# jwang1x/VT-precondition

Measured on AMD Instinct MI355X. Metric: precond-GMRES iters/sec + CSR SpMV achieved-HBM-GB/s, 1/2/4/8 MI355X, higher is better.
Workload: dtype f64; 1 GPU; C3: GMRES(20, auto)+BJ(8) to rtol=1e-08, n=20000000, row-sharded over 1 GPU(s); n=20000000, nnz=99950000, restart=20, prec=bj, bs=8, operator=generated, line_band=800, bj_apply=tridiag, layout=sell, orth=auto, parallelism=row-slab x1

## Files before the change

vt-precondition_amd/csrc/vtk_band.hip:

```cpp
#include <hip/hip_runtime.h>

#include <algorithm>
#include <cstdlib>

#include "vtk_device.hpp"

namespace vtk {


#define VTK_BAND_DOTS_UNROLL 2
constexpr int BAND_XUP_XB = 4;
constexpr int BAND_PF = 12;

template <int OPT> constexpr int band_wpe() { return (OPT & 2) ? 6 : 4; }
__device__ __forceinline__ int band_block(int opt, int H) {
    const int b = blockIdx.x;
    if (!(opt & 4) || H != 2 || (gridDim.x & 15) != 0) return b;
    return (((b >> 4) << 3) + (b & 7)) * 2 + ((b >> 3) & 1);
}
__device__ __forceinline__ double band_msub(double acc, double a, double b) { return __builtin_fma(-a, b, acc); }
__device__ __forceinline__ double band_madd(double acc, double a, double b) { return __builtin_fma(a, b, acc); }
template <int OPT> __device__ __forceinline__ void band_sync() {
    if constexpr (OPT & 8) asm volatile("s_waitcnt lgkmcnt(0)\n\ts_barrier" ::: "memory");
    else __syncthreads();
}
constexpr int BAND_OFF = 16;
static_assert(BAND_LP + 2 * BAND_OFF <= BAND_T && BAND_OFF % 8 == 0, "band geometry");
template <int WU, int J, int VMODE = 0, bool GH = true, int OPT = 0>
__global__ __launch_bounds__(BAND_T) __attribute__((amdgpu_waves_per_eu(band_wpe<OPT>()))) void k_band_step(BandK a) {
    constexpr int BAND_RS = BAND_T;
    constexpr int BAND_W = BAND_T / 64, BAND_IT = (J + 2 + BAND_W - 1) / BAND_W;
    __shared__ double vbuf[(J + 1) * BAND_LP];
    __shared__ double ring[4 * BAND_RS];
    __shared__ double wbuf[BAND_LP];
    __shared__ double red[DC_NQ];
    __shared__ double cs[BAND_JV], ce[BAND_JV], cp[BAND_JV];
    __shared__ int pf_sink[64];
    constexpr int j = J;
    if (__builtin_nontemporal_load(&a.st->xup_tag) == j) {
        dc_xupdate_body<BAND_XUP_XB, true>(a.V, a.ld, j, __builtin_nontemporal_load(&a.st->stop_col), a.n, a.cf, a.x,
                                           a.H, a.S, a.m, a.w_prev);
        return;
    }
    if (stopped(&a.st->stop_col, j)) return;
    const int tid = threadIdx.x, lane = tid & 63, wv = tid >> 6;
    const int L = a.L, X = a.X, H = a.H_parts, LP = L / H;
    const int b = band_block(a.opt, H), R = (int)gridDim.x / H, rb = b / H, h = b % H, v0 = h * LP;
    const int xa = (int)((int64_t)rb * X / R), xb = (int)((int64_t)(rb + 1) * X / R);
    const int v = v0 - BAND_OFF + tid;
    const int wrapL = (X - 1) * L;
    const bool own = tid >= BAND_OFF && tid < BAND_OFF + LP;
    const bool upd = tid >= BAND_OFF - 1 && tid <= LP + BAND_OFF && v >= 0 && v < L;
    constexpr bool LSV = VMODE >= 1, CANON = VMODE == 2;
    const int ii = lane & 7;
    double tx0 = 0.0, tx1 = 0.0;
    if constexpr (LSV) {
        if (v >= 0 && v < L) {
            tx0 = a.lsv[a.n + v];
            tx1 = a.lsv[a.n + L + v];
        }
    }
    for (int k = tid; k < j; k += BAND_T) {
        cs[k] = a.cf->s[k];
        ce[k] = a.cf->e[k];
        cp[k] = a.cf->e_prev[k];
    }
    const double rinv = a.cf->rinv, qc = a.cf->q, ej = a.cf->e[j], qp = a.cf->q_prev;
    band_sync<OPT>();
    double vreg[J + 1];
    double acc[BAND_IT][3];
#pragma unroll
    for (int u = 0; u < BAND_IT; ++u) acc[u][0] = acc[u][1] = acc[u][2] = 0.0;
    const int nl = xb - xa;
    const int xhm = xa == 0 ? X - 1 : xa - 1, xhp = xb == X ? 0 : xb;
    const bool rev = ((a.opt & 16) && (rb & 1)) != ((a.opt & 32) && (J & 1));
    auto line_of = [&](int it, int &kind) {
        if (rev) {
            kind = it == 0 ? 2 : (it == nl + 1 ? 1 : 0);
            return it == 0 ? xhp : (it == nl + 1 ? xhm : xb - it);
        }
        kind = it == 0 ? 1 : (it == nl + 1 ? 2 : 0);
        return it == 0 ? xhm : (it == nl + 1 ? xhp : xa - 1 + it);
    };
    auto spmv_line = [&](int it) { return rev ? xb + 1 - it : xa - 2 + it; };
    constexpr bool PF = J <= BAND_PF;
    constexpr bool SPF = PF && CANON && (OPT & 1);
    struct Ld {
        double v[J > 0 ? J : 1];
        double wm, wj;
        double drow, mrow, tv0, tv1;
    };
    auto load = [&](int it, Ld &o) {
        int kind;
        const int y = line_of(it, kind);
        if constexpr (SPF) {
            o.drow = 0.0;
            o.mrow = 1.0;
            o.tv0 = o.tv1 = 0.0;
            if (it >= 2) {
                const int xs = spmv_line(it);
                const int64_t rs = (int64_t)xs * L + (own ? v : v0);
                if (own) {
                    o.drow = __builtin_nontemporal_load(a.lsv + rs);
                    o.mrow = __builtin_nontemporal_load(a.mtri + rs);
                }
                o.tv0 = a.lsv[a.n + 2 * L + xs];
                o.tv1 = a.lsv[a.n + 2 * L + X + xs];
            }
        }
        const int64_t row = (int64_t)y * L + (upd ? v : 0);
        o.wm = 0.0;
        o.wj = 0.0;
        const double *gh = (GH && a.ghost && ((kind == 1 && rb == 0) || (kind == 2 && rb == R - 1)))
                               ? a.ghost + (size_t)(kind == 1 ? 0 : 1) * (a.m + 2) * L : nullptr;
        if (upd) {
            if (gh) {
                o.wj = gh[(size_t)(a.m + (j & 1)) * L + v];
                o.wm = gh[(size_t)(j == 0 ? 0 : a.m + ((j + 1) & 1)) * L + v];
            } else {
                o.wj = __builtin_nontemporal_load(a.w_in + row);
                o.wm = __builtin_nontemporal_load((j == 0 ? a.V : a.w_prev) + row);
            }
        }
        if (gh) {
#pragma unroll
            for (int k = 0; k < J; ++k) o.v[k] = upd ? gh[(size_t)k * L + v] : 0.0;
        } else {
            const double *pv = a.V + row;
#pragma unroll
            for (int k = 0; k < J; ++k) {
                o.v[k] = upd ? __builtin_nontemporal_load(pv) : 0.0;
                pv += a.ld;
            }
        }
    };
    auto update = [&](int it, const Ld &o) -> double {
        int kind;
        const int y = line_of(it, kind);
        const int64_t row = (int64_t)y * L + (upd ? v : 0);
#pragma unroll
        for (int k = 0; k < J; ++k) vreg[k] = o.v[k];
        double pj = o.wm;
        if (j >= 1) {
            double tp = o.wm;
#pragma unroll
            for (int k = 0; k < J; ++k) tp = band_msub(tp, cp[k], vreg[k]);
            pj = tp * qp;
        }
        double av = pj, tv = o.wj;
#pragma unroll
        for (int k = 0; k < J; ++k) {
            const double sk = cs[k], ek = ce[k];
            av = band_msub(av, sk, vreg[k]);
            tv = band_msub(tv, ek, vreg[k]);
        }
        double vj = pj;
        if (j >= 1) vj = av * rinv;
        tv = band_msub(tv, ej, vj);
        const double pn = tv * qc;
        vreg[J] = vj;
        if (kind == 0 && own) {
            if (j >= 1) {
                st_wt(a.V + (size_t)j * a.ld + row, vj);
            }
            if (j == a.m - 2) st_wt(a.V + (size_t)(j + 1) * a.ld + row, pn);
        }
        return pn;
    };
    auto stage = [&](double *vb) {
        if (own) {
#pragma unroll
            for (int k = 0; k <= J; ++k) vb[k * BAND_LP + tid - BAND_OFF] = vreg[k];
        }
    };
    auto slot = [&](int y) { return ((y - xa + 1) & 3) * BAND_RS; };
    constexpr int PF_ROWS = J + 2 + (CANON ? 2 : 0);
    auto l2_prefetch = [&](int itp) {
        if constexpr ((OPT & 8) != 0) {
            if (itp > nl + 1) return;
            int kind;
            const int y = line_of(itp, kind);
            const bool ghostl = GH && a.ghost && ((kind == 1 && rb == 0) || (kind == 2 && rb == R - 1));
            const int xs = spmv_line(itp);
            const int vlo = v0 > 0 ? v0 - 1 : 0, vhi = v0 + LP < L ? v0 + LP + 1 : L;
            for (int r = wv; r < PF_ROWS; r += BAND_W) {
                const double *vec;
                int64_t r0, r1;
                if (r < J + 2) {
                    if (ghostl) continue;
                    vec = r < J ? a.V + (size_t)r * a.ld : (r == J ? a.w_in : (j == 0 ? a.V : a.w_prev));
                    r0 = (int64_t)y * L + vlo;
                    r1 = (int64_t)y * L + vhi;
                } else {
                    if (itp < 2) continue;
                    vec = r == J + 2 ? a.lsv : a.mtri;
                    r0 = (int64_t)xs * L + v0;
                    r1 = r0 + LP;
                }
                const int64_t s0 = r0 >> 4, ns = ((r1 - 1) >> 4) - s0 + 1;
                if (lane < ns)
                    __builtin_amdgcn_global_load_lds(vec + ((s0 + lane) << 4), (__attribute__((address_space(3))) void *)pf_sink,
                                                     4, 0, 0);
            }
        }
    };
    Ld nx;
    if constexpr (PF) load(0, nx);
    l2_prefetch(PF ? 1 : 0);
    for (int it = 0; it <= nl + 1; ++it) {
        const int y = rev ? xb - it : xa - 1 + it, x = spmv_line(it);
        const bool work = it >= 2;
        const int64_t lrow = (int64_t)(work ? x : xa) * L;
        const int64_t row = lrow + (own ? v : v0);
        const int64_t q = row >> 6, q0 = (lrow + v0 - BAND_OFF + 64 * wv) >> 6;
        const int l64 = (int)(row & 63);
        uint32_t word = 0u;
        int dv = 0;
        double d[LSV ? 1 : WU];
        double mrow = 1.0, drow = 0.0, tv0 = 0.0, tv1 = 0.0;
        if (work && !SPF) {
            if constexpr (!CANON) {
                word = __builtin_nontemporal_load(a.pk + q * 64 + l64);
                const int64_t qd = q0 + (lane >> 4);
                dv = (lane < 32 && qd >= 0 && qd * 64 < a.n) ? a.dict[qd * 16 + (lane & 15)] : 0;
            }
            if constexpr (LSV) {
                if (own) drow = __builtin_nontemporal_load(a.lsv + row);
                tv0 = a.lsv[a.n + 2 * L + x];
                tv1 = a.lsv[a.n + 2 * L + X + x];
            } else {
#pragma unroll
                for (int k = 0; k < WU; ++k) d[k] = __builtin_nontemporal_load(a.val + q * 64 * WU + 64 * k + l64);
            }
            if (own) mrow = __builtin_nontemporal_load(a.mtri + row);
        }
        {
            Ld cu;
            if constexpr (PF) cu = nx;
            else load(it, cu);
            if constexpr (SPF) {
                drow = cu.drow;
                mrow = cu.mrow;
                tv0 = cu.tv0;
                tv1 = cu.tv1;
            }
            const double pn = update(it, cu);
            if (upd) ring[slot(y) + tid] = pn;
            if constexpr (PF) {
                if (it <= nl) load(it + 1, nx);
            }
            l2_prefetch(PF ? it + 2 : it + 1);
        }
        band_sync<OPT>();
        if (work) {
            double sacc = 0.0, sub = 0.0, sup = 0.0;
            if constexpr (CANON) {
                int64_t cxm, cxp;
                const int ord = __builtin_amdgcn_readfirstlane(
                    canon_order_xv(x, 0, a.n, L, X, GH && a.ghost ? a.left_blk : -1, cxm, cxp, a.xord));
                const int sx = ((x - xa + 1) & 3) * BAND_RS - v0 + BAND_OFF;
                constexpr int P_MID = 0 | 1 << 3 | 2 << 6 | 3 << 9 | 4 << 12;
                constexpr int P_FIRST = 1 | 2 << 3 | 3 << 6 | 4 << 9 | 0 << 12;
                constexpr int P_LAST = 4 | 0 << 3 | 1 << 6 | 2 << 9 | 3 << 12;
                const bool sl = a.canon == 2 && (ord == P_MID || ord == P_FIRST || ord == P_LAST);
                if (sl) {
                    const int vv = own ? v : v0;
                    const double t0 = tx0 * ring[((x - xa) & 3) * BAND_RS - v0 + BAND_OFF + vv];
                    const double t4 = tx1 * ring[((x - xa + 2) & 3) * BAND_RS - v0 + BAND_OFF + vv];
                    const double t2 = drow * ring[sx + vv];
                    const double t1 = tv0 * ring[sx + vv - 1];
                    const double t3 = tv1 * ring[sx + vv + 1];
                    const bool h1 = vv > 0, h3 = vv < L - 1;
                    double sa = 0.0;
                    if (ord == P_MID) {
                        sa = sa + t0;
                        sa = h1 ? sa + t1 : sa;
                        sa = sa + t2;
                        sa = h3 ? sa + t3 : sa;
                        sa = sa + t4;
                    } else if (ord == P_FIRST) {
                        sa = h1 ? sa + t1 : sa;
                        sa = sa + t2;
                        sa = h3 ? sa + t3 : sa;
                        sa = sa + t4;
                        sa = sa + t0;
                    } else {
                        sa = sa + t4;
                        sa = sa + t0;
                        sa = h1 ? sa + t1 : sa;
                        sa = sa + t2;
                        sa = h3 ? sa + t3 : sa;
                    }
                    sacc = own ? sa : 0.0;
                    sub = (own && h1 && ii > 0) ? 0.0 + tv0 : 0.0;
                    sup = (own && h3 && ii < 7) ? 0.0 + tv1 : 0.0;
                }
#pragma unroll
                for (int e = 0; e < 5; ++e) {
                    const int kind = (ord >> (3 * e)) & 7;
                    if (!sl && own) {
                        if (kind == 0) sacc += tx0 * ring[((x - xa) & 3) * BAND_RS - v0 + BAND_OFF + v];
                        else if (kind == 4) sacc += tx1 * ring[((x - xa + 2) & 3) * BAND_RS - v0 + BAND_OFF + v];
                        else if (kind == 2) sacc += drow * ring[sx + v];
                        else if (kind == 1) {
                            if (v > 0) {
                                sacc += tv0 * ring[sx + v - 1];
                                if (ii > 0) sub = sub + tv0;
                            }
                        } else if (v < L - 1) {
                            sacc += tv1 * ring[sx + v + 1];
                            if (ii < 7) sup = sup + tv1;
                        }
                    }
                }
            } else {
                const int sel = (int)(q - q0) * 16;
#pragma unroll
                for (int k = 0; k < WU; ++k) {
                    const int code = (int)((word >> (4 * k)) & 15u);
                    const int off = __shfl(dv, (sel + code) & 63, 64);
                    if (own && code != PK_CODES) {
                        const int t = v + off;
                        int rel, vc;
                        const int c = x * L + t;
                        if (a.ghost && c >= (int)a.n) {
                            const int kk = c - (int)a.n, blk = kk >= L ? 1 : 0;
                            rel = blk == a.left_blk ? -1 : 1;
                            vc = kk - blk * L;
                        } else if (t >= 0 && t < L) { rel = 0; vc = t; }
                        else if (t >= L && t < 2 * L) { rel = 1; vc = t - L; }
                        else if (t < 0 && t >= -L) { rel = -1; vc = t + L; }
                        else if (t >= L) { rel = -1; vc = t - wrapL; }
                        else { rel = 1; vc = t + wrapL; }
                        const double xv = ring[((x - xa + 1 + rel) & 3) * BAND_RS + vc - v0 + BAND_OFF];
                        double dk;
                        if constexpr (LSV) dk = rel != 0 ? (rel > 0 ? tx1 : tx0) : (vc == v ? drow : (vc > v ? tv1 : tv0));
                        else dk = d[k];
                        sacc += dk * xv;
                        if (off == -1 && ii > 0) sub = sub + dk;
                        if (off == 1 && ii < 7) sup = sup + dk;
                    }
                }
            }
            const double z = bj_trim_group<8>(own ? sacc : 0.0, lane, sub, sup, mrow);
            if (own) {
                st_wt(a.w_out + row, z);
                wbuf[tid - BAND_OFF] = z;
            }
            band_sync<OPT>();
            const double *pr = ring + slot(x) + BAND_OFF;
#pragma unroll
            for (int u = 0; u < BAND_IT; ++u) {
                const int itm = wv + BAND_W * u;
                if (itm <= j) {
                    const double *vk = vbuf + itm * BAND_LP;
#pragma unroll VTK_BAND_DOTS_UNROLL
                    for (int t = lane; t < LP; t += 64) {
                        const double vv = vk[t];
                        acc[u][0] = band_madd(acc[u][0], vv, pr[t]);
                        acc[u][1] = band_madd(acc[u][1], vv, wbuf[t]);
                    }
                } else if (itm == j + 1) {
#pragma unroll VTK_BAND_DOTS_UNROLL
                    for (int t = lane; t < LP; t += 64) {
                        const double pv = pr[t], wq = wbuf[t];
                        acc[u][0] = band_madd(acc[u][0], pv, pv);
                        acc[u][1] = band_madd(acc[u][1], pv, wq);
                        acc[u][2] = band_madd(acc[u][2], wq, wq);
                    }
                }
            }
            band_sync<OPT>();
        }
        if (it >= 1 && it <= nl) stage(vbuf);
    }
#pragma unroll
    for (int u = 0; u < BAND_IT; ++u) {
        const int itm = wv + BAND_W * u;
        if (itm <= j + 1) {
            const double t0 = wave_allsum(acc[u][0]), t1 = wave_allsum(acc[u][1]), t2 = wave_allsum(acc[u][2]);
            if (lane == 0) {
                if (itm <= j) {
                    red[itm] = t0;
                    red[DC_MAXJ + itm] = t1;
                } else {
                    red[2 * DC_MAXJ] = t0;
                    red[2 * DC_MAXJ + 1] = t1;
                    red[2 * DC_MAXJ + 2] = t2;
                }
            }
        }
    }
    __syncthreads();
    const int jn = j + 1;
    for (int qq = tid; qq < DC_NQ; qq += BAND_T) {
        const bool used = qq < jn || (qq >= DC_MAXJ && qq < DC_MAXJ + jn) || qq >= 2 * DC_MAXJ;
        if (used) a.part[(size_t)qq * GMAX + b] = red[qq];
    }
}

template <int J> constexpr bool band_spf_j() { return J == 0 || J == 3 || J == 4; }
template <int J> static void launch_band_one_rank(const BandK &a0, int grid, hipStream_t s) {
    BandK a = a0;
    if constexpr (!band_spf_j<J>()) a.opt &= ~1;
    const dim3 g(grid), blk(BAND_T);
    if constexpr (J > BAND_PF) {
        if (a.opt & 8) { hipLaunchKernelGGL((k_band_step<5, J, 2, false, 9>), g, blk, 0, s, a); return; }
    }
    if constexpr (J <= BAND_J3) {
        if ((a.opt & 3) == 3) { hipLaunchKernelGGL((k_band_step<5, J, 2, false, 3>), g, blk, 0, s, a); return; }
        if ((a.opt & 3) == 2) { hipLaunchKernelGGL((k_band_step<5, J, 2, false, 2>), g, blk, 0, s, a); return; }
    }
    if (a.opt & 1) hipLaunchKernelGGL((k_band_step<5, J, 2, false, 1>), g, blk, 0, s, a);
    else hipLaunchKernelGGL((k_band_step<5, J, 2, false>), g, blk, 0, s, a);
}

template <int J> static void launch_band_ghost(const BandK &a0, int grid, hipStream_t s) {
    BandK a = a0;
    if constexpr (!band_spf_j<J>()) a.opt &= ~1;
    const dim3 g(grid), blk(BAND_T);
    if constexpr (J > BAND_PF) {
        if (a.opt & 8) { hipLaunchKernelGGL((k_band_step<5, J, 2, true, 9>), g, blk, 0, s, a); return; }
    }
    if constexpr (J <= BAND_J3) {
        if ((a.opt & 3) == 3) { hipLaunchKernelGGL((k_band_step<5, J, 2, true, 3>), g, blk, 0, s, a); return; }
        if ((a.opt & 3) == 2) { hipLaunchKernelGGL((k_band_step<5, J, 2, true, 2>), g, blk, 0, s, a); return; }
    }
    if constexpr (J > BAND_J3 && J <= BAND_PF) {
        if (a.opt & 1) { hipLaunchKernelGGL((k_band_step<5, J, 2, true, 1>), g, blk, 0, s, a); return; }
    }
    hipLaunchKernelGGL((k_band_step<5, J, 2>), g, blk, 0, s, a);
}

hipError_t launch_band_step(const BandK &a, int grid, int wu, hipStream_t s) {
    if (wu != 5 || a.H_parts < 1 || a.L % a.H_parts != 0 || a.L / a.H_parts > BAND_LP || (a.L / a.H_parts) % 8 != 0 ||
        a.j + 1 > BAND_JV || grid < a.H_parts || grid > GMAX || grid % a.H_parts != 0 || grid / a.H_parts > a.X ||
        a.n > INT32_MAX / 2)
        return hipErrorInvalidValue;
    switch (a.j) {
#define VTK_BAND_J(J_)                                                                                           \
    case J_:                                                                                                     \
        if (a.lsv && a.canon && !a.ghost) launch_band_one_rank<J_>(a, grid, s); \
        else if (a.lsv && a.canon) launch_band_ghost<J_>(a, grid, s); \
        else if (a.lsv) hipLaunchKernelGGL((k_band_step<5, J_, 1>), dim3(grid), dim3(BAND_T), 0, s, a); \
        else hipLaunchKernelGGL((k_band_step<5, J_>), dim3(grid), dim3(BAND_T), 0, s, a); \
        break;
        VTK_BAND_J(0) VTK_BAND_J(1) VTK_BAND_J(2) VTK_BAND_J(3) VTK_BAND_J(4) VTK_BAND_J(5) VTK_BAND_J(6)
        VTK_BAND_J(7) VTK_BAND_J(8) VTK_BAND_J(9) VTK_BAND_J(10) VTK_BAND_J(11) VTK_BAND_J(12) VTK_BAND_J(13)
        VTK_BAND_J(14) VTK_BAND_J(15) VTK_BAND_J(16) VTK_BAND_J(17) VTK_BAND_J(18)
#undef VTK_BAND_J
        default: return hipErrorInvalidValue;
    }
    return hipGetLastError();
}

__global__ __launch_bounds__(NT) void k_ghost_pack(const double *__restrict__ V, int64_t ld, int j,
                                                   const double *__restrict__ w, int64_t n, int L,
                                                   double *__restrict__ sbuf, int64_t off_first, int64_t off_last) {
    constexpr int NV = BAND_GHOST_VECS;
    for (int i = blockIdx.x * NT + threadIdx.x; i < 2 * NV * L; i += gridDim.x * NT) {
        const int side = i / (NV * L), r = i % (NV * L), vec = r / L, t = r % L;
        const int64_t off = side == 0 ? off_first : off_last;
        if (off < 0) continue;
        const int64_t row = (side == 0 ? 0 : n - L) + t;
        sbuf[off + r] = vec == 0 ? V[(size_t)(j >= 1 ? j - 1 : 0) * ld + row] : w[row];
    }
}

__global__ __launch_bounds__(NT) void k_ghost_unpack(const double *__restrict__ rbuf, int64_t off_left, int64_t off_right,
                                                     int j, int m, int L, double *__restrict__ ghost) {
    constexpr int NV = BAND_GHOST_VECS;
    for (int i = blockIdx.x * NT + threadIdx.x; i < 2 * NV * L; i += gridDim.x * NT) {
        const int side = i / (NV * L), r = i % (NV * L), vec = r / L, t = r % L;
        const int64_t off = side == 0 ? off_left : off_right;
        if (off < 0) continue;
        const int slot = vec == 0 ? (j >= 1 ? j - 1 : 0) : m + (j & 1);
        ghost[((size_t)side * (m + 2) + slot) * L + t] = rbuf[off + r];
    }
}

hipError_t launch_ghost_pack(const double *V, int64_t ld, int j, const double *w, int64_t n, int L, double *sbuf,
                             int64_t off_first, int64_t off_last, hipStream_t s) {
    hipLaunchKernelGGL(k_ghost_pack, dim3((2 * BAND_GHOST_VECS * L + NT - 1) / NT), dim3(NT), 0, s, V, ld, j, w, n, L, sbuf, off_first,
                       off_last);
    return hipGetLastError();
}

hipError_t launch_ghost_unpack(const double *rbuf, int64_t off_left, int64_t off_right, int j, int m, int L,
                               double *ghost, hipStream_t s) {
    hipLaunchKernelGGL(k_ghost_unpack, dim3((2 * BAND_GHOST_VECS * L + NT - 1) / NT), dim3(NT), 0, s, rbuf, off_left, off_right, j, m, L,
                       ghost);
    return hipGetLastError();
}

__global__ __launch_bounds__(NT) void k_band_check_dist(const int32_t *__restrict__ indptr,
                                                        const int32_t *__restrict__ indices, int64_t n, int L,
                                                        int lblk, int *bad) {
    const int64_t X = n / L;
    for (int64_t r = (int64_t)blockIdx.x * NT + threadIdx.x; r < n; r += (int64_t)gridDim.x * NT) {
        const int64_t x = r / L, vr = r % L;
        bool ok = true, vloc = true;
        for (int k = indptr[r]; k < indptr[r + 1]; ++k) {
            const int64_t c = indices[k];
            int64_t vc;
            if (c < 0 || c >= n + 2 * L) { ok = false; break; }
            if (c < n) {
                const int64_t rel = c / L - x;
                if (rel < -1 || rel > 1) { ok = false; break; }
                vc = c % L;
            } else {
                const int64_t kk = c - n, blk = kk / L;
                if ((blk == lblk && x != 0) || (blk != lblk && x != X - 1)) { ok = false; break; }
                vc = kk % L;
            }
            if (vc - vr < -1 || vc - vr > 1) vloc = false;
        }
        if (!ok) atomicOr(bad, 1);
        if (!vloc) atomicOr(bad, 2);
    }
}

hipError_t launch_band_check_dist(const int32_t *indptr, const int32_t *indices, int64_t n, int L, int lblk, int *bad,
                                  hipStream_t s) {
    int64_t g = (n + NT - 1) / NT;
    if (g > 4096) g = 4096;
    if (g < 1) g = 1;
    hipLaunchKernelGGL(k_band_check_dist, dim3((unsigned)g), dim3(NT), 0, s, indptr, indices, n, L, lblk, bad);
    return hipGetLastError();
}

__device__ __forceinline__ int lsv_slot(int64_t r, int64_t c, int64_t n, int L, int X, int lblk, int64_t &idx) {
    const int64_t x = r / L, v = r % L;
    int64_t dx, vc;
    if (c < n) {
        dx = c / L - x;
        vc = c % L;
        if (lblk < 0) {
            if (dx == X - 1) dx = -1;
            else if (dx == -(X - 1)) dx = 1;
        }
    } else {
        const int64_t kk = c - n, blk = kk / L;
        dx = blk == lblk ? -1 : 1;
        vc = kk % L;
    }
    if (dx == 0) {
        if (vc == v) { idx = r; return 0; }
        if (vc == v - 1 || vc == v + 1) { idx = (int64_t)n + 2 * L + (vc > v ? X : 0) + x; return 2; }
        return -1;
    }
    if ((dx == 1 || dx == -1) && vc == v) { idx = (int64_t)n + (dx > 0 ? L : 0) + v; return 1; }
    return -1;
}

__global__ __launch_bounds__(NT) void k_lsv_build(const int32_t *__restrict__ indptr, const int32_t *__restrict__ indices,
                                                  const double *__restrict__ data, int64_t n, int L, int lblk,
                                                  int xord, double *__restrict__ lsv, int *bad, int pass) {
    const int X = (int)(n / L);
    for (int64_t r = (int64_t)blockIdx.x * NT + threadIdx.x; r < n; r += (int64_t)gridDim.x * NT) {
        for (int k = indptr[r]; k < indptr[r + 1]; ++k) {
            int64_t idx;
            if (lsv_slot(r, indices[k], n, L, X, lblk, idx) < 0) {
                atomicOr(bad, 1);
                break;
            }
            if (pass == 0) lsv[idx] = data[k];
            else if (__double_as_longlong(lsv[idx]) != __double_as_longlong(data[k])) atomicOr(bad, 1);
        }
        if (pass == 1) {
            int64_t cxm, cxp;
            const int ord = canon_order(r, n, L, X, lblk, cxm, cxp, xord);
            const int64_t v = r % L;
            int k = indptr[r];
            bool ok = true;
            for (int e = 0; e < 5 && ok; ++e) {
                const int kind = (ord >> (3 * e)) & 7;
                if ((kind == 1 && v == 0) || (kind == 3 && v == L - 1)) continue;
                const int64_t c = kind == 0 ? cxm : (kind == 4 ? cxp : r + kind - 2);
                ok = k < indptr[r + 1] && indices[k] == c;
                ++k;
            }
            if (!ok || k != indptr[r + 1]) atomicOr(bad, 2);
        }
    }
}

hipError_t launch_lsv_build(const int32_t *indptr, const int32_t *indices, const double *data, int64_t n, int L,
                            int lblk, int xord, double *lsv, int *bad, hipStream_t s) {
    if (L <= 0 || n % L != 0 || n / L < 2) return hipErrorInvalidValue;
    int64_t g = (n + NT - 1) / NT;
    if (g > 4096) g = 4096;
    if (g < 1) g = 1;
    for (int pass = 0; pass < 2; ++pass) {
        hipLaunchKernelGGL(k_lsv_build, dim3((unsigned)g), dim3(NT), 0, s, indptr, indices, data, n, L, lblk, xord, lsv, bad, pass);
        const hipError_t e = hipGetLastError();
        if (e != hipSuccess) return e;
    }
    return hipSuccess;
}

template <typename VT>
__global__ __launch_bounds__(NT) void k_grid4_build(const int32_t *__restrict__ indptr, const int32_t *__restrict__ indices,
                                                    const VT *__restrict__ data, int64_t n, Grid4 g,
                                                    double *__restrict__ tab, VT *__restrict__ D, int *bad, int pass) {
    for (int64_t r = (int64_t)blockIdx.x * NT + threadIdx.x; r < n; r += (int64_t)gridDim.x * NT) {
        const G4Row q = g4_coords(r, g);
        int64_t c[9];
        bool p[9];
        g4_cols(r, q, g, n, c, p);
        int64_t key[9];
        for (int k = 0; k < 9; ++k) key[k] = k == 0 || k == 8 ? g4_key(c[k], k, n, g) : c[k];
        int ord[9], m = 0;
        for (int k = 0; k < 9; ++k)
            if (p[k]) ord[m++] = k;
        for (int i = 1; i < m; ++i)
            for (int t = i; t > 0 && key[ord[t]] < key[ord[t - 1]]; --t) {
                const int s = ord[t];
                ord[t] = ord[t - 1];
                ord[t - 1] = s;
            }
        const int k0 = indptr[r];
        bool ok = indptr[r + 1] - k0 == m;
        for (int e = 0; e < m && ok; ++e) {
            const int kind = ord[e];
            if ((int64_t)indices[k0 + e] != c[kind] || (e > 0 && c[ord[e]] == c[ord[e - 1]])) { ok = false; break; }
            const VT dv = data[k0 + e];
            if (kind == 4) {
                if (pass == 0) D[r] = dv;
            } else {
                const int sl = g4_slot(kind, q, g);
                if (pass == 0) tab[sl] = (double)dv;
                else if (__double_as_longlong(tab[sl]) != __double_as_longlong((double)dv)) ok = false;
            }
        }
        if (!ok) atomicOr(bad, 1);
    }
}

hipError_t launch_grid4_build(const int32_t *indptr, const int32_t *indices, const void *data, int fp32, int64_t n,
                              const Grid4 &g, double *tab, void *D, int *bad, hipStream_t s) {
    const int64_t S4 = (int64_t)g.Ny * g.Nvx * g.Nvy;
    if (g.Ny < 3 || g.Nvx < 2 || g.Nvy < 2 || S4 <= 0 || n % S4 != 0 || n / S4 != g.X || n > INT32_MAX / 2 ||
        (g.lblk < 0 && g.X < 3))
        return hipErrorInvalidValue;
    int64_t gr = (n + NT - 1) / NT;
    if (gr > 4096) gr = 4096;
    if (gr < 1) gr = 1;
    for (int pass = 0; pass < 2; ++pass) {
        if (fp32) hipLaunchKernelGGL(k_grid4_build<float>, dim3((unsigned)gr), dim3(NT), 0, s, indptr, indices,
                                     (const float *)data, n, g, tab, (float *)D, bad, pass);
        else hipLaunchKernelGGL(k_grid4_build<double>, dim3((unsigned)gr), dim3(NT), 0, s, indptr, indices,
                                (const double *)data, n, g, tab, (double *)D, bad, pass);
        const hipError_t e = hipGetLastError();
        if (e != hipSuccess) return e;
    }
    return hipSuccess;
}

template <bool HALO, bool CANON = false>
__global__ __launch_bounds__(NT) void k_lsv_spmv(const uint32_t *__restrict__ pk, const int32_t *__restrict__ dict,
                                                 const double *__restrict__ lsv, const double *__restrict__ x,
                                                 const double *__restrict__ halo, double *__restrict__ y, int n, int L,
                                                 int lblk, int xord, const int *stop_col, int col) {
    if (stopped(stop_col, col)) return;
    const int lane = threadIdx.x & 63;
    const int X = n / L, nch = (n + 63) >> 6;
    for (int q = (int)(((int64_t)blockIdx.x * NT + threadIdx.x) >> 6); q < nch; q += (int)((int64_t)gridDim.x * NT >> 6)) {
        const int r = 64 * q + lane;
        const bool act = r < n;
        int xl = (64 * q) / L, v = 64 * q - xl * L + lane;
        while (v >= L) {
            v -= L;
            ++xl;
        }
        const double drow = act ? __builtin_nontemporal_load(lsv + r) : 0.0;
        double s = 0.0;
        if constexpr (CANON) {
            if (act) {
                int c[5];
                double d[5];
                canon_row(lsv, n, L, lblk, xl, v, drow, c, d, xord);
                double xv[5];
#pragma unroll
                for (int k = 0; k < 5; ++k) {
                    const int cc = c[k] >= 0 ? c[k] : r;
                    xv[k] = (HALO && cc >= n) ? halo[cc - n] : x[cc];
                }
#pragma unroll
                for (int k = 0; k < 5; ++k)
                    if (c[k] >= 0) s += d[k] * xv[k];
                __builtin_nontemporal_store(s, y + r);
            }
            continue;
        }
        const uint32_t word = act ? __builtin_nontemporal_load(pk + (size_t)q * 64 + lane) : ~0u;
        const int dv = lane < 16 ? dict[(size_t)q * 16 + lane] : 0;
#pragma unroll
        for (int k = 0; k < 5; ++k) {
            const int code = (int)((word >> (4 * k)) & 15u);
            const int off = __shfl(dv, code, 64);
            if (act && code != PK_CODES) {
                const int c = r + off;
                double val;
                if (off == 0) val = drow;
                else if (off == 1 || off == -1) val = lsv[(size_t)n + 2 * L + (off > 0 ? X : 0) + xl];
                else {
                    const bool up = (HALO && c >= n) ? ((c - n) / L != lblk) : (off == L || (lblk < 0 && off == -(X - 1) * L));
                    val = lsv[(size_t)n + (up ? L : 0) + v];
                }
                const double xv = (HALO && c >= n) ? halo[c - n] : x[c];
                s += val * xv;
            }
        }
        if (act) __builtin_nontemporal_store(s, y + r);
    }
}

__global__ __launch_bounds__(BAND_T) void k_lsv_ring(const double *__restrict__ lsv, const double *__restrict__ x,
                                                     double *__restrict__ y, int n, int L, int H, const int *stop_col,
                                                     int col) {
    __shared__ double ring[4 * BAND_T];
    if (stopped(stop_col, col)) return;
    const int tid = threadIdx.x, X = n / L, LP = L / H;
// ... 531 lines not shown
```

vt-precondition_amd/csrc/vtk_internal.hpp:

```cpp
#pragma once
#include <cmath>
#include <hip/hip_runtime.h>
#include <rccl/rccl.h>
#include <stdint.h>

#include <string>
#include <vector>

#include "../../include/vtkrylov.h"

namespace vtk {

constexpr int NT = 256;
constexpr int TILE_ROWS = 512;
constexpr int TILE_NNZ = 4096;
constexpr int GMAX = 1024;
constexpr int MAX_RESTART = 1024;
constexpr int BIG_COL = 1 << 30;

struct GmresState {
    double ptol;
    double presid;
    double rnorm;
    double scal[8];
    int stop_col;
    int breakdown;
    long long inner;
    int xup_tag;
    int pad_;
};

constexpr int DC_MAXJ = 32;
constexpr int DC_NQ = 2 * DC_MAXJ + 3;
constexpr int DC_VOTE = DC_NQ;
constexpr int DC_NQV = DC_NQ + 1;
constexpr int PEER_FAILED = 2;
struct DcCoef {
    double s[DC_MAXJ];
    double e[DC_MAXJ + 1];
    double rinv;
    double q;
    double nu;
    double h0[DC_MAXJ + 1];
    int committed[DC_MAXJ + 1];
    double e_prev[DC_MAXJ + 1];
    double q_prev;
};

struct Red {
    const double *p;
    int cnt;
};

struct Tiles {
    int32_t *d_row = nullptr;
    int32_t *d_end = nullptr;
    int ntiles = 0;
    int align = 1;
    bool has_long = false;
    bool aligned = true;
    int grid = 0;
    int64_t nrows = 0;
};

struct Sell {
    int64_t *d_off = nullptr;
    int32_t *d_col = nullptr;
    void *d_val = nullptr;
    int64_t nch = 0, entries = 0;
    uint32_t *d_pk = nullptr;
    int64_t *d_pkoff = nullptr;
    int32_t *d_dict = nullptr;
    int64_t n_wide = 0;
    int64_t wide_entries = 0;
    int64_t pk_words = 0;
    int uniform_w = 0;
};
constexpr int PK_CODES = 15;

struct Groups {
    int32_t *d_list = nullptr;
    int count = 0;
    int grid = 0;
};

struct LineOp {
    double *f = nullptr;
    int64_t n = 0, row0 = 0, stride = 1, seg = 1;
    int64_t i_lo = 0, i_hi = -1;
    int64_t nseg = 0;
    int64_t j0 = 0, jn = 0;
    int64_t jb = 0;
    double *ac = nullptr;
    int compact = 0;
};

struct Grid4 {
    int Ny = 0, Nvx = 0, Nvy = 0, X = 0;
    int lblk = -1;
    int xord = 0;
    const double *tab = nullptr;
    const void *D = nullptr;
};
inline size_t grid4_tab_len(const Grid4 &g) { return 2 * ((size_t)g.Nvx + g.Nvy + g.X + g.Ny); }
constexpr int G4TAB = 1024;
constexpr int G4RM = 64;
inline int g4_ring_group(int gr) { return gr >= 512 ? 512 : 256; }
inline int64_t g4_ring_per(int64_t ng, int64_t S4, int G, int wgs) {
    const int64_t per0 = std::max<int64_t>(1, (ng + std::max(1, wgs) - 1) / std::max(1, wgs));
    const double gpp = (double)S4 / G;
    if (gpp < 8.0 || gpp / (double)per0 > 32.0) return per0;
    const int64_t q = std::max<int64_t>(8, (int64_t)std::ceil(gpp / (double)per0 / 8.0) * 8);
    return std::max<int64_t>(1, std::llround(gpp / (double)q));
}
inline bool g4_ring_fits(const Grid4 &g, int64_t n, int gr) {
    const int64_t S3 = (int64_t)g.Nvx * g.Nvy;
    return n > 0 && n <= INT32_MAX / 2 && 2 * S3 + 2 * g4_ring_group(gr) <= 8192 && grid4_tab_len(g) <= (size_t)G4TAB &&
           g.Nvy < G4RM;
}

struct Tuning {
    int band = 1;
    int band_lsv = 1;
    int sell_canon = 1;
    int band_canon = 1;
    int band_opt = 63;
    int band_long_rows = 16000000;
    int lsv_ring = 2048;
    int prof_perj = 0;
    int comm_solo = 0;
    int auto_band = 1;
    int grid4 = 1;
    int c4_fused = 1;
    int g4_ring = 2048;
    int g4_gr = 512;
    int g4_fast = 1;
    int line_fuse = 1;
    int cyc_ring = 512;
    int fail_step = -1;
};
}

struct vtk_ctx {
    int device = 0;
    hipStream_t stream = nullptr;
    hipStream_t comm_stream = nullptr;
    hipEvent_t ev_pack = nullptr, ev_halo = nullptr;
    std::string err;
    int rank = 0, world = 1;
    bool dist = false;
    ncclComm_t comm = nullptr;
    bool host_comm = false;
    bool comm_broken = false;
    vtk_host_comm hops{};
    int orth = VTK_ORTH_AUTO;
    vtk::Tuning tune;
    int n_cu = 0;
    double *d_part = nullptr;
    double *d_scal = nullptr;
    vtk::GmresState *d_state = nullptr;
    vtk::GmresState *h_state = nullptr;
    int *h_stop = nullptr;
    int *d_stop = nullptr;
    void *ws = nullptr;
    size_t ws_bytes = 0;
    struct ProfPending { int cls; int col; double bytes; hipEvent_t e0, e1; };
    struct ProfAcc { std::string name; int64_t launches = 0; double seconds = 0, bytes = 0; };
    bool prof_on = false;
    std::vector<ProfPending> prof_pending;
    std::vector<ProfAcc> prof_acc;
    std::vector<hipEvent_t> prof_pool;
};

struct vtk_csr {
    vtk_ctx *ctx = nullptr;
    int device = 0;
    int64_t n_global = 0, row_begin = 0, row_end = 0, n_local = 0, nnz = 0;
    int fp32 = 0;
    int32_t *d_indptr = nullptr, *d_indices = nullptr;
    void *d_data = nullptr;
    std::vector<int32_t> h_indptr;
    std::vector<uint8_t> row_halo;
    vtk::Sell sell;
    bool use_sell = false;
    int layout = VTK_LAYOUT_AUTO;
    vtk::Groups g_all, g_in, g_bd;
    std::vector<int64_t> offsets;
    vtk::Tiles tiles;
    int64_t n_halo = 0;
    std::vector<int64_t> halo_cols;
    std::vector<int64_t> recv_cnt, recv_off;
    std::vector<int64_t> send_cnt, send_off;
    double *d_halo = nullptr;
    int32_t *d_send_idx = nullptr;
    double *d_send_buf = nullptr;
    int64_t n_send = 0;
    int64_t band_L = 0;
    bool band_vloc = false;
    double *d_lsv = nullptr;
    bool lsv_canon = false;
    vtk::Grid4 g4;
    double *d_g4tab = nullptr;
    void *d_g4D = nullptr;
    bool band_ghost = false;
    int band_lblk = 0;
    int band_xord = 0;
    int band_peer[2] = {-1, -1};
    std::vector<int64_t> band_scnt, band_soff, band_rcnt, band_roff;
    int64_t band_off_first = -1, band_off_last = -1;
    int64_t band_off_left = -1, band_off_right = -1;
    int64_t values_epoch = 0;
    bool from_vlasov = false;
    vtk_vlasov_params vparams{};
    vtk::Grid4 g4_try;
};

struct vtk_prec {
    vtk_csr *A = nullptr;
    int device = 0;
    int bs = 8;
    int64_t nb = 0;
    double *d_inv = nullptr;
    vtk::Tiles tiles;
    bool fused = false;
    vtk::Tiles tiles_in, tiles_bd;
    bool split = false;
    double *d_tri = nullptr;
    int64_t tri_ld = 0;
    bool tri_ok = false;
    int mode = VTK_BJ_AUTO;
    int kind = VTK_PREC_BJACOBI;
    vtk::LineOp line;
    bool line_compact_ok = false;
    int setup = VTK_BJ_SETUP_EXACT;
    int compact_req = -1;
    int64_t epoch = 0;
    bool valid = true;
};

namespace vtk {

struct SpmvIn {
    const int32_t *indptr, *indices;
    const void *data;
    int fp32;
    const Tiles *tiles;
    int n_local;
    const double *x, *halo;
    const Sell *sell = nullptr;
    const Groups *groups = nullptr;
    const double *lsv = nullptr;
    int lsv_L = 0, lsv_lblk = -1;
    int lsv_xord = 0;
    int lsv_canon = 0;
    int plain_grid = 0;
    Grid4 g4{};
    int swz = 0;
    int plain_var = 0;
};

LineOp line_plan(int64_t n, int64_t row0, int64_t stride, int64_t seg);

struct BjOp {
    const double *inv = nullptr;
    const double *tri = nullptr;
    int64_t tri_ld = 0;
    int bs = 0;
    const LineOp *line = nullptr;
};

hipError_t launch_index_range(const int32_t *idx, int64_t n, int *mm, hipStream_t s);

inline int spmv_grid(const SpmvIn &in) { return (in.sell && in.groups) ? in.groups->grid : in.tiles->grid; }

enum Epi { EPI_PLAIN = 0, EPI_RESID = 1, EPI_PREC = 2, EPI_RESID_PREC = 3, EPI_PREC_DC = 4 };

hipError_t launch_spmv(const SpmvIn &in, int epi, double *y, const double *b, const BjOp &bj,
                       const double *v0, double *part0, double *part1,
                       const int *stop_col, int col, hipStream_t s);
hipError_t launch_bj_apply(const BjOp &bj, int64_t n, const double *r, double *z,
                           const double *v0, double *part0, double *part1, int grid,
                           const int *stop_col, int col, hipStream_t s);
hipError_t launch_sell_build(const int32_t *indptr, const int32_t *indices, const void *data, int fp32, int64_t n,
                             int64_t *off, int64_t *tmp64, void *scan_tmp, size_t scan_bytes, int32_t *col,
                             void *val, int phase, hipStream_t s);
size_t sell_scan_bytes(int64_t n);
hipError_t launch_sell_pack(const int64_t *off, int64_t nch, int64_t *pkoff, int64_t *tmp64, void *scan_tmp,
                            size_t scan_bytes, const int32_t *col, uint32_t *pk, int32_t *dict,
                            unsigned long long *wide_cnt, int phase, hipStream_t s);
hipError_t launch_line_setup(const int32_t *indptr, const int32_t *indices, const void *data, int fp32,
                             const LineOp &L, unsigned long long *bad_row, unsigned long long *ext, hipStream_t s);
hipError_t launch_line_dc(const LineOp &L, const double *r, double *w, const double *V, int64_t ld, int j,
                          const double *p, double *part, int grid, const int *stop_col, int col, hipStream_t s);
hipError_t launch_line_spmv_dc(const LineOp &L, const double *lsv, const double *p, double *w, const double *V,
                               int64_t ld, int j, double *part, int grid, const int *stop_col, int col, hipStream_t s);
hipError_t launch_line_apply(const LineOp &L, const double *r, double *z, const double *v0, double *part0,
                             double *part1, int grid, const int *stop_col, int col, hipStream_t s);
hipError_t launch_bj_tri_setup(const int32_t *indptr, const int32_t *indices, const void *data, int fp32,
                               int64_t n, int bs, const double *inv, double *tri, int64_t ld, int *flags,
                               hipStream_t s);
hipError_t launch_bj_setup(const int32_t *indptr, const int32_t *indices, const void *data,
                           int fp32, int64_t n, int bs, double *inv, int *d_singular,
                           double *work, hipStream_t s);
hipError_t launch_bj_setup_mfma(const int32_t *indptr, const int32_t *indices, const void *data, int fp32, int64_t n,
                                int bs, double *inv, int *d_singular, hipStream_t s);
hipError_t launch_mgs(Red hin, double *hout, double *w, const double *vk, const double *vnext,
                      int64_t n, double *part_out, int grid, const int *stop_col, int col,
                      hipStream_t s);
hipError_t launch_tail(Red h0, Red w2, const double *w, double *vnext, int64_t n, int col,
                       int m, double *H, double *S, double *giv, GmresState *st, int *stop_map,
                       int grid, hipStream_t s);
hipError_t launch_scale0(Red p, double *v0, int64_t n, double *S, int m, GmresState *st,
                         int grid, hipStream_t s);
hipError_t launch_xupdate(const double *H, const double *S, const double *V, int64_t ld,
                          double *x, int64_t n, int m, const GmresState *st, int grid, hipStream_t s);
hipError_t launch_finalize(Red p, double *dst, int do_sqrt, hipStream_t s);
hipError_t launch_dot(const double *x, const double *y, int64_t n, double *part, int grid,
                      hipStream_t s);
hipError_t launch_any_nonzero(const double *x, int64_t n, double *flag, hipStream_t s);
hipError_t launch_gather(const double *x, const int32_t *idx, int64_t cnt, double *out,
                         hipStream_t s);
hipError_t launch_vlasov_counts(const vtk_vlasov_params &p, int64_t r0, int64_t nrows,
                                int32_t *counts, hipStream_t s);
hipError_t launch_vlasov_fill(const vtk_vlasov_params &p, int64_t r0, int64_t nrows,
                              const int32_t *indptr, int32_t *indices, void *data,
                              hipStream_t s);
hipError_t launch_sell_refresh(const int32_t *indptr, const void *data, int fp32, int64_t n, const int64_t *off,
                               void *val, hipStream_t s);
hipError_t launch_vlasov_values(const vtk_vlasov_params &p, int64_t r0, int64_t nrows, const int32_t *indptr,
                                void *data, hipStream_t s);
hipError_t launch_exclusive_scan(const int32_t *in, int32_t *out, int64_t n, void *tmp,
                                 size_t *tmp_bytes, hipStream_t s);
hipError_t launch_remap_cols(int32_t *indices, int64_t nnz, int64_t row_begin, int64_t n_local,
                             const int64_t *halo_cols, int64_t n_halo, hipStream_t s);

hipError_t launch_dc_dots(const double *V, int64_t ld, int j, const double *w, int64_t n,
                          double *part, int grid, const int *stop_col, int col, hipStream_t s);
hipError_t launch_spmv_dc(const SpmvIn &in, double *w, const BjOp &bj, const double *V,
                          int64_t ld, int j, double *part, const int *stop_col, int col, hipStream_t s);
hipError_t launch_dc_finalize(const double *part, int cnt, int j, int with_w, double *scal,
                              const int *stop_col, int col, hipStream_t s);
hipError_t launch_dc_scalar(const double *part, int cnt, const double *scal, int j, int m,
                            int closing, double *Hraw, double *H, double *S, double *giv,
                            DcCoef *cf, GmresState *st, int *stop_map, hipStream_t s);
hipError_t launch_dc_update(double *V, int64_t ld, int j, const double *w, int64_t n,
                            const DcCoef *cf, int grid, const GmresState *st, double *x,
                            const double *H, const double *S, int m, int nt_pw, hipStream_t s);

struct BandK {
    const uint32_t *pk;
    const int32_t *dict;
    const double *val;
    const double *mtri;
    double *V;
    int64_t ld;
    int j, m;
    const double *w_in;
    const double *w_prev;
    double *w_out;
    const DcCoef *cf;
    const GmresState *st;
    double *x;
    const double *H, *S;
    double *part;
    int64_t n;
    int L, X, H_parts;
    const double *ghost;
    int left_blk;
    int xord = 0;
    const double *lsv;
    int canon;
    int opt = 0;
};
hipError_t launch_band_step(const BandK &a, int grid, int wu, hipStream_t s);
constexpr int BAND_LP = 400, BAND_T = 448, BAND_WPC = 2;
constexpr int BAND_JV = 19;
constexpr int BAND_J3 = 2;
constexpr int BAND_GHOST_VECS = 2;
hipError_t launch_band_check_dist(const int32_t *indptr, const int32_t *indices, int64_t n, int L, int lblk, int *bad,
                                  hipStream_t s);
hipError_t launch_ghost_pack(const double *V, int64_t ld, int j, const double *w, int64_t n, int L, double *sbuf,
                             int64_t off_first, int64_t off_last, hipStream_t s);
hipError_t launch_ghost_unpack(const double *rbuf, int64_t off_left, int64_t off_right, int j, int m, int L,
                               double *ghost, hipStream_t s);
int band_parts(int64_t L, int lp = BAND_LP);
hipError_t launch_lsv_build(const int32_t *indptr, const int32_t *indices, const double *data, int64_t n, int L,
                            int lblk, int xord, double *lsv, int *bad, hipStream_t s);
hipError_t launch_lsv_ring_epi(int epi, const double *lsv, const double *x, const double *b, const double *mtri,
                               double *y, double *p0, double *p1, double *dcpart, int64_t n, int L, int ring_wgs,
                               const int *stop_col, int col, int *grid_out, hipStream_t s, const double *halo = nullptr,
                               int lblk = -1, int xord = 0);
hipError_t launch_lsv_spmv(const uint32_t *pk, const int32_t *dict, const double *lsv, const double *x,
                           const double *halo, double *y, int64_t n, int L, int lblk, const int *stop_col, int col,
                           hipStream_t s, int canon, int grid_cap,
                           int ring_wgs = 0, int xord = 0);
hipError_t launch_grid4_build(const int32_t *indptr, const int32_t *indices, const void *data, int fp32, int64_t n,
                              const Grid4 &g, double *tab, void *D, int *bad, hipStream_t s);
struct G4Dots {
    int mode = 2;
    double *part = nullptr;
    const double *b = nullptr;
    double *p0 = nullptr, *p1 = nullptr;
    int part_off = 0;
};
hipError_t launch_g4_ring(const Grid4 &g, const double *x, const double *halo, const double *mtri, double *w, int64_t n,
                          int fp32, int wgs, int gr, const G4Dots *dots, int *grid_out, const int *stop_col,
                          int col, hipStream_t s, int g_lo = 0, int g_hi = -1, int per = 0, int fast = 1);
hipError_t launch_band_check(const int32_t *indptr, const int32_t *indices, int64_t n, int L, int X, int *bad,
                             hipStream_t s);

int vector_grid(int64_t n);

void build_tiles(const std::vector<int32_t> &indptr, int align, std::vector<int32_t> &rows,
                 bool &has_long, bool &aligned);
void set_context_free_error(const std::string &msg);

}
```

Before: 1818 iters/s.

## Split band-step prefetch and dot passes into thirds for large Krylov columns

```diff
diff --git a/vt-precondition_amd/csrc/vtk_band.hip b/vt-precondition_amd/csrc/vtk_band.hip
--- a/vt-precondition_amd/csrc/vtk_band.hip
+++ b/vt-precondition_amd/csrc/vtk_band.hip
@@ -2,6 +2,7 @@
 
 #include <algorithm>
 #include <cstdlib>
+#include <type_traits>
 
 #include "vtk_device.hpp"
 
@@ -21,7 +22,7 @@
 __device__ __forceinline__ double band_msub(double acc, double a, double b) { return __builtin_fma(-a, b, acc); }
 __device__ __forceinline__ double band_madd(double acc, double a, double b) { return __builtin_fma(a, b, acc); }
 template <int OPT> __device__ __forceinline__ void band_sync() {
-    if constexpr (OPT & 8) asm volatile("s_waitcnt lgkmcnt(0)\n\ts_barrier" ::: "memory");
+    if constexpr (OPT & (8 | 64)) asm volatile("s_waitcnt lgkmcnt(0)\n\ts_barrier" ::: "memory");
     else __syncthreads();
 }
 constexpr int BAND_OFF = 16;
@@ -84,7 +85,10 @@
     };
     auto spmv_line = [&](int it) { return rev ? xb + 1 - it : xa - 2 + it; };
     constexpr bool PF = J <= BAND_PF;
-    constexpr bool SPF = PF && CANON && (OPT & 1);
+    constexpr bool TH = J > BAND_PF && (OPT & 64) != 0;
+    static_assert(!TH || BAND_IT == 3, "thirds: three dots passes");
+    constexpr int TH_G0 = BAND_W, TH_G1 = BAND_W, TH_G2 = TH ? J + 2 - TH_G0 - TH_G1 : 1;
+    constexpr bool SPF = CANON && ((PF && (OPT & 1)) || TH);
     struct Ld {
         double v[J > 0 ? J : 1];
         double wm, wj;
@@ -134,6 +138,52 @@
             }
         }
     };
+    const uint32_t vo_upd = (uint32_t)(upd ? v : 0) * 8u, vo_own = (uint32_t)(own ? v : v0) * 8u;
+    auto lane_at = [](auto *line, uint32_t vo) {
+        asm volatile("" : "+v"(vo));
+        return (decltype(line))((const char *)line + vo);
+    };
+    auto load_spf = [&](int it, double &drow, double &mrow, double &tv0, double &tv1) {
+        drow = 0.0;
+        mrow = 1.0;
+        tv0 = tv1 = 0.0;
+        if (it >= 2) {
+            const int xs = spmv_line(it);
+            const int64_t ls = (int64_t)xs * L;
+            if (own) {
+                drow = __builtin_nontemporal_load(lane_at(a.lsv + ls, vo_own));
+                mrow = __builtin_nontemporal_load(lane_at(a.mtri + ls, vo_own));
+            }
+            tv0 = a.lsv[a.n + 2 * L + xs];
+            tv1 = a.lsv[a.n + 2 * L + X + xs];
+        }
+    };
+    auto load_part = [&](int it, auto LO, auto HI, double *dst) {
+        constexpr int lo = decltype(LO)::value, hi = decltype(HI)::value;
+        int kind;
+        const int y = line_of(it, kind);
+        const double *gh = (GH && a.ghost && ((kind == 1 && rb == 0) || (kind == 2 && rb == R - 1)))
+                               ? a.ghost + (size_t)(kind == 1 ? 0 : 1) * (a.m + 2) * L : nullptr;
+        if (gh) {
+#pragma unroll
+            for (int k = lo; k < hi; ++k) {
+                const size_t sl = k < J ? (size_t)k : (size_t)(k == J ? a.m + (j & 1) : (j == 0 ? 0 : a.m + ((j + 1) & 1)));
+                dst[k - lo] = upd ? *lane_at(gh + sl * L, vo_upd) : 0.0;
+            }
+        } else {
+            const double *pv = a.V + (int64_t)y * L + (int64_t)lo * a.ld;
+#pragma unroll
+            for (int k = lo; k < hi; ++k) {
+                if (k < J) {
+                    dst[k - lo] = upd ? __builtin_nontemporal_load(lane_at(pv, vo_upd)) : 0.0;
+                    pv += a.ld;
+                } else {
+                    const double *pw = (k == J ? a.w_in : (j == 0 ? a.V : a.w_prev)) + (int64_t)y * L;
+                    dst[k - lo] = upd ? __builtin_nontemporal_load(lane_at(pw, vo_upd)) : 0.0;
+                }
+            }
+        }
+    };
     auto update = [&](int it, const Ld &o) -> double {
         int kind;
         const int y = line_of(it, kind);
@@ -160,10 +210,16 @@
         const double pn = tv * qc;
         vreg[J] = vj;
         if (kind == 0 && own) {
-            if (j >= 1) {
-                st_wt(a.V + (size_t)j * a.ld + row, vj);
-            }
-            if (j == a.m - 2) st_wt(a.V + (size_t)(j + 1) * a.ld + row, pn);
+            if constexpr (TH) {
+                double *vl = a.V + (size_t)j * a.ld + (int64_t)y * L;
+                st_wt(lane_at(vl, vo_upd), vj);
+                if (j == a.m - 2) st_wt(lane_at(vl + a.ld, vo_upd), pn);
+            } else {
+                if (j >= 1) {
+                    st_wt(a.V + (size_t)j * a.ld + row, vj);
+                }
+                if (j == a.m - 2) st_wt(a.V + (size_t)(j + 1) * a.ld + row, pn);
+            }
         }
         return pn;
     };
@@ -171,6 +227,13 @@
         if (own) {
 #pragma unroll
             for (int k = 0; k <= J; ++k) vb[k * BAND_LP + tid - BAND_OFF] = vreg[k];
+        }
+    };
+    auto stage_part = [&](auto LO, auto HI) {
+        constexpr int lo = decltype(LO)::value, hi = decltype(HI)::value;
+        if (own) {
+#pragma unroll
+            for (int k = lo; k < hi; ++k) vbuf[k * BAND_LP + tid - BAND_OFF] = vreg[k];
         }
     };
     auto slot = [&](int y) { return ((y - xa + 1) & 3) * BAND_RS; };
@@ -204,8 +267,45 @@
             }
         }
     };
+    auto dots_pass = [&](int x, auto U) {
+        constexpr int u = decltype(U)::value;
+        const double *pr = ring + slot(x) + BAND_OFF;
+        const int itm = wv + BAND_W * u;
+        if (BAND_W * (u + 1) <= J + 1 || itm <= j) {
+            const double *vk = vbuf + itm * BAND_LP;
+#pragma unroll VTK_BAND_DOTS_UNROLL
+            for (int t = lane; t < LP; t += 64) {
+                const double vv = vk[t];
+                acc[u][0] = band_madd(acc[u][0], vv, pr[t]);
+                acc[u][1] = band_madd(acc[u][1], vv, wbuf[t]);
+            }
+        } else if ((J + 1) / BAND_W == u && itm == j + 1) {
+#pragma unroll VTK_BAND_DOTS_UNROLL
+            for (int t = lane; t < LP; t += 64) {
+                const double pv = pr[t], wq = wbuf[t];
+                acc[u][0] = band_madd(acc[u][0], pv, pv);
+                acc[u][1] = band_madd(acc[u][1], pv, wq);
+                acc[u][2] = band_madd(acc[u][2], wq, wq);
+            }
+        }
+    };
     Ld nx;
     if constexpr (PF) load(0, nx);
+    double g0[TH_G0], g1[TH_G1], g2[TH_G2];
+    double sd = 0.0, sm = 1.0, st0 = 0.0, st1 = 0.0;
+    using I0 = std::integral_constant<int, 0>;
+    using I1 = std::integral_constant<int, TH_G0>;
+    using I2 = std::integral_constant<int, TH_G0 + TH_G1>;
+    using I3 = std::integral_constant<int, J + 2>;
+    using S1 = std::integral_constant<int, BAND_W>;
+    using S2 = std::integral_constant<int, 2 * BAND_W>;
+    using IJ = std::integral_constant<int, J + 1>;
+    if constexpr (TH) {
+        load_part(0, I0{}, I1{}, g0);
+        load_spf(0, sd, sm, st0, st1);
+        load_part(0, I1{}, I2{}, g1);
+        load_part(0, I2{}, I3{}, g2);
+    }
     l2_prefetch(PF ? 1 : 0);
     for (int it = 0; it <= nl + 1; ++it) {
         const int y = rev ? xb - it : xa - 1 + it, x = spmv_line(it);
@@ -236,7 +336,17 @@
         }
         {
             Ld cu;
-            if constexpr (PF) cu = nx;
+            if constexpr (TH) {
+                auto opnd = [&](int k) { return k < TH_G0 ? g0[k] : (k < TH_G0 + TH_G1 ? g1[k - TH_G0] : g2[k - TH_G0 - TH_G1]); };
+#pragma unroll
+                for (int k = 0; k < J; ++k) cu.v[k] = opnd(k);
+                cu.wj = opnd(J);
+                cu.wm = opnd(J + 1);
+                cu.drow = sd;
+                cu.mrow = sm;
+                cu.tv0 = st0;
+                cu.tv1 = st1;
+            } else if constexpr (PF) cu = nx;
             else load(it, cu);
             if constexpr (SPF) {
                 drow = cu.drow;
@@ -248,6 +358,12 @@
             if (upd) ring[slot(y) + tid] = pn;
             if constexpr (PF) {
                 if (it <= nl) load(it + 1, nx);
+            }
+            if constexpr (TH) {
+                if (it <= nl) {
+                    load_part(it + 1, I0{}, I1{}, g0);
+                    load_spf(it + 1, sd, sm, st0, st1);
+                }
             }
             l2_prefetch(PF ? it + 2 : it + 1);
         }
@@ -344,35 +460,59 @@
             }
             const double z = bj_trim_group<8>(own ? sacc : 0.0, lane, sub, sup, mrow);
             if (own) {
-                st_wt(a.w_out + row, z);
+                if constexpr (TH) st_wt(lane_at(a.w_out + lrow, vo_own), z);
+                else st_wt(a.w_out + row, z);
                 wbuf[tid - BAND_OFF] = z;
             }
             band_sync<OPT>();
-            const double *pr = ring + slot(x) + BAND_OFF;
-#pragma unroll
-            for (int u = 0; u < BAND_IT; ++u) {
-                const int itm = wv + BAND_W * u;
-                if (itm <= j) {
-                    const double *vk = vbuf + itm * BAND_LP;
+            if constexpr (!TH) {
+                const double *pr = ring + slot(x) + BAND_OFF;
+#pragma unroll
+                for (int u = 0; u < BAND_IT; ++u) {
+                    const int itm = wv + BAND_W * u;
+                    if (itm <= j) {
+                        const double *vk = vbuf + itm * BAND_LP;
 #pragma unroll VTK_BAND_DOTS_UNROLL
-                    for (int t = lane; t < LP; t += 64) {
-                        const double vv = vk[t];
-                        acc[u][0] = band_madd(acc[u][0], vv, pr[t]);
-                        acc[u][1] = band_madd(acc[u][1], vv, wbuf[t]);
-                    }
-                } else if (itm == j + 1) {
+                        for (int t = lane; t < LP; t += 64) {
+                            const double vv = vk[t];
+                            acc[u][0] = band_madd(acc[u][0], vv, pr[t]);
+                            acc[u][1] = band_madd(acc[u][1], vv, wbuf[t]);
+                        }
+                    } else if (itm == j + 1) {
 #pragma unroll VTK_BAND_DOTS_UNROLL
-                    for (int t = lane; t < LP; t += 64) {
-                        const double pv = pr[t], wq = wbuf[t];
-                        acc[u][0] = band_madd(acc[u][0], pv, pv);
-                        acc[u][1] = band_madd(acc[u][1], pv, wq);
-                        acc[u][2] = band_madd(acc[u][2], wq, wq);
+                        for (int t = lane; t < LP; t += 64) {
+                            const double pv = pr[t], wq = wbuf[t];
+                            acc[u][0] = band_madd(acc[u][0], pv, pv);
+                            acc[u][1] = band_madd(acc[u][1], pv, wq);
+                            acc[u][2] = band_madd(acc[u][2], wq, wq);
+                        }
                     }
                 }
-            }
-            band_sync<OPT>();
-        }
-        if (it >= 1 && it <= nl) stage(vbuf);
+                band_sync<OPT>();
+            }
+        }
+        if constexpr (TH) {
+            const bool stg = it >= 1 && it <= nl, ldn = it <= nl;
+            if (work) {
+                dots_pass(x, I0{});
+                band_sync<OPT>();
+            }
+            if (stg) stage_part(I0{}, S1{});
+            if (ldn) load_part(it + 1, I1{}, I2{}, g1);
+            if (work) {
+                dots_pass(x, std::integral_constant<int, 1>{});
+                band_sync<OPT>();
+            }
+            if (stg) stage_part(S1{}, S2{});
+            if (ldn) load_part(it + 1, I2{}, I3{}, g2);
+            if (work) {
+                dots_pass(x, std::integral_constant<int, 2>{});
+                band_sync<OPT>();
+            }
+            if (stg) stage_part(S2{}, IJ{});
+        } else {
+            if (it >= 1 && it <= nl) stage(vbuf);
+        }
     }
 #pragma unroll
     for (int u = 0; u < BAND_IT; ++u) {
@@ -400,11 +540,13 @@
 }
 
 template <int J> constexpr bool band_spf_j() { return J == 0 || J == 3 || J == 4; }
+template <int J> constexpr bool band_thirds_ghost_j() { return J == 13 || J == 14 || J == 16; }
 template <int J> static void launch_band_one_rank(const BandK &a0, int grid, hipStream_t s) {
     BandK a = a0;
     if constexpr (!band_spf_j<J>()) a.opt &= ~1;
     const dim3 g(grid), blk(BAND_T);
     if constexpr (J > BAND_PF) {
+        if (a.opt & 64) { hipLaunchKernelGGL((k_band_step<5, J, 2, false, 64>), g, blk, 0, s, a); return; }
         if (a.opt & 8) { hipLaunchKernelGGL((k_band_step<5, J, 2, false, 9>), g, blk, 0, s, a); return; }
     }
     if constexpr (J <= BAND_J3) {
@@ -419,6 +561,9 @@
     BandK a = a0;
     if constexpr (!band_spf_j<J>()) a.opt &= ~1;
     const dim3 g(grid), blk(BAND_T);
+    if constexpr (band_thirds_ghost_j<J>()) {
+        if (a.opt & 64) { hipLaunchKernelGGL((k_band_step<5, J, 2, true, 64>), g, blk, 0, s, a); return; }
+    }
     if constexpr (J > BAND_PF) {
         if (a.opt & 8) { hipLaunchKernelGGL((k_band_step<5, J, 2, true, 9>), g, blk, 0, s, a); return; }
     }
diff --git a/vt-precondition_amd/csrc/vtk_internal.hpp b/vt-precondition_amd/csrc/vtk_internal.hpp
--- a/vt-precondition_amd/csrc/vtk_internal.hpp
+++ b/vt-precondition_amd/csrc/vtk_internal.hpp
@@ -124,7 +124,7 @@
     int band_lsv = 1;
     int sell_canon = 1;
     int band_canon = 1;
-    int band_opt = 63;
+    int band_opt = 127;
     int band_long_rows = 16000000;
     int lsv_ring = 2048;
     int prof_perj = 0;
```

After: 1849 iters/s, median of 6. +1.7%, better.
